# VISION-SJTU/VEON

Measured on AMD Instinct MI355X. Metric: 6cam_lift_samples_per_sec, higher is better.
Workload: dtype f32; 1 GPU; S2: 6-cam 256x704, D=59, C=80, 200x200x16 voxels, view_transform(accelerate=True) -> (B,C,Z,Y,X); points_kept=108978, intervals=72699, launch=eager, output_volume=allocator-placed (torch.empty per step), parallelism=replicas x1 (one sample per GPU, no collective)

## Files before the change

include/veon_hip.h:

```cpp
#ifndef VEON_HIP_H_
#define VEON_HIP_H_

#include <stddef.h>
#include <stdint.h>

#ifdef __cplusplus
extern "C" {
#endif

#define VEON_ABI_VERSION 2

#define VEON_OK 0
#define VEON_ERR_BAD_ARG 1
#define VEON_ERR_LAUNCH 2
#define VEON_ERR_WORKSPACE 3

#define VEON_LAYOUT_BZYXC 0
#define VEON_LAYOUT_BCZYX 1

#define VEON_FEAT_F32 0
#define VEON_FEAT_F16 1
#define VEON_FEAT_BF16 2


int veon_abi_version(void);
int veon_half_mode(void);
const char *veon_status_string(int status);

int veon_bev_pool_v2_fwd(int c, int n_intervals, const float *depth,
                         const float *feat, const int *ranks_depth,
                         const int *ranks_feat, const int *ranks_bev,
                         const int *interval_starts,
                         const int *interval_lengths, float *out, void *stream);

int veon_bev_pool_v2_bwd(int c, int n_intervals, const float *out_grad,
                         const float *depth, const float *feat,
                         const int *ranks_depth, const int *ranks_feat,
                         const int *ranks_bev, const int *interval_starts,
                         const int *interval_lengths, float *depth_grad,
                         float *feat_grad, void *stream);

int veon_bev_pool_tile_voxels(void);
int64_t veon_bev_pool_plan_ints(int batch, int64_t voxels_per_batch);
int veon_bev_pool_plan(int n_intervals, int n_points, int batch,
                       int64_t voxels_per_batch, const int *ranks_bev,
                       const int *interval_starts, const int *counts, int *plan,
                       void *stream);

int veon_bev_pool_v2_fwd_fused(int c, int n_intervals, int batch,
                               int64_t voxels_per_batch, const float *depth,
                               const float *feat, const int *ranks_depth,
                               const int *ranks_feat, const int *ranks_bev,
                               const int *interval_starts,
                               const int *interval_lengths, const int *plan,
                               float *out, int out_layout, void *stream);

int veon_bev_pool_row_table(int n_intervals, int n_points, int batch,
                            int64_t voxels_per_batch, int row_voxels,
                            const int *ranks_bev, const int *interval_starts,
                            const int *counts, int *row_first, int *row_point,
                            void *stream);
int veon_bev_pool_v2_fwd_maxpool(int c, int n_intervals, int batch, int Z, int Y,
                                 int X, int dz, int dy, int dx,
                                 const float *depth, const float *feat,
                                 const int *ranks_depth, const int *ranks_feat,
                                 const int *ranks_bev,
                                 const int *interval_starts,
                                 const int *interval_lengths,
                                 const int *row_first, float *out,
                                 void *stream);

int veon_bev_pool_v2_fwd_fused_ex(int c, int n_intervals, int batch,
                                  int64_t voxels_per_batch, const float *depth,
                                  const void *feat, int feat_dtype,
                                  const int *ranks_depth, const int *ranks_feat,
                                  const int *ranks_bev,
                                  const int *interval_starts,
                                  const int *interval_lengths, const int *plan,
                                  float *out, int out_layout, void *stream);
int veon_bev_pool_v2_fwd_maxpool_ex(int c, int n_intervals, int batch, int Z,
                                    int Y, int X, int dz, int dy, int dx,
                                    const float *depth, const void *feat,
                                    int feat_dtype, const int *ranks_depth,
                                    const int *ranks_feat, const int *ranks_bev,
                                    const int *interval_starts,
                                    const int *interval_lengths,
                                    const int *row_first, float *out,
                                    void *stream);

int veon_bev_pool_v2_fwd_fused_strided(int c, int n_intervals, int batch,
                                       int64_t voxels_per_batch, const float *depth,
                                       const void *feat, int feat_dtype,
                                       const int *ranks_depth, const int *ranks_feat,
                                       const int *ranks_bev,
                                       const int *interval_starts,
                                       const int *interval_lengths, const int *plan,
                                       float *out, int64_t plane_stride,
                                       void *stream);

int veon_feat_nchw_to_nhwc(const void *in, void *out, int elem_bytes, int images,
                           int C, int HW, void *stream);

int veon_bev_pool_v2_fwd_maxpool_padded(int c, int n_intervals, int batch, int Z,
                                        int Y, int X, int dz, int dy, int dx,
                                        const float *depth, const void *feat,
                                        int feat_dtype, const int *ranks_depth,
                                        const int *ranks_feat,
                                        const int *ranks_bev,
                                        const int *interval_starts,
                                        const int *interval_lengths,
                                        const int *row_first,
                                        void *out_padded_bf16, void *stream);

int veon_volume_maxpool2_f32(const float *in, float *out, int64_t planes, int Z, int Y,
                             int X, void *stream);


int64_t veon_bev_pool_voxel_table_ints(int batch, int64_t voxels_per_batch);
int veon_bev_pool_voxel_table(int n_intervals, int n_points, int batch,
                              int64_t voxels_per_batch, const int *ranks_bev,
                              const int *interval_starts, const int *counts,
                              int *vstart, void *stream);
int veon_bev_pool_v2_fwd_rows(int c, int batch, int64_t voxels_per_batch,
                              const float *depth, const void *feat, int feat_dtype,
                              const int *ranks_depth, const int *ranks_feat,
                              const int *vstart, float *out, int64_t plane_stride,
                              int64_t feat_elems, int variant, void *stream);
int veon_bev_pool_v2_fwd_rows_maxpool(int c, int batch, int Z, int Y, int X, int dz,
                                      int dy, int dx, const float *depth,
                                      const void *feat, int feat_dtype,
                                      const int *ranks_depth, const int *ranks_feat,
                                      const int *vstart, void *out, int out_padded_bf16,
                                      int64_t feat_elems, void *stream);

int veon_bev_pool_rows_maxpool_chunk(void);
int veon_bev_pool_v2_fwd_rows_maxpool_ordered(
    int c, int batch, int Z, int Y, int X, int dz, int dy, int dx, const float *depth,
    const void *feat, int feat_dtype, const int *ranks_depth, const int *ranks_feat,
    const int *vstart, void *out, int out_padded_bf16, int64_t feat_elems,
    const int *chunk_order, void *stream);

int veon_bev_pool_v2_fwd_rows_maxpool_winner(
    int c, int batch, int Z, int Y, int X, int dz, int dy, int dx, const float *depth,
    const void *feat, int feat_dtype, const int *ranks_depth, const int *ranks_feat,
    const int *vstart, void *out, int64_t feat_elems, const int *chunk_order,
    uint8_t *winner, void *stream);
int veon_bev_pool_point_table(int n_points, int64_t table_len, int64_t n_voxels,
                              const int *ranks_depth, const int *ranks_bev,
                              const int *counts, int *pvox, void *stream);
int veon_bev_pool_v2_bwd_rows_maxpool(int c, int n_images, int D, int HW, int batch, int Z,
                                      int Y, int X, const float *pooled_grad,
                                      const uint8_t *winner, const int *pvox,
                                      const float *depth, const float *feat,
                                      float *depth_grad, float *feat_grad, void *stream);


int veon_camera_matrices(int BN, const float *sensor2ego, const float *cam2imgs,
                         const float *post_rots, float *post_rots_inv,
                         float *combine, float *trans, void *stream);

int veon_lidar_coor(int B, int N, int D, int H, int W, const float *xs,
                    const float *ys, const float *ds,
                    const float *post_rots_inv, const float *post_trans,
                    const float *combine, const float *trans, const float *bda,
                    float *coor, void *stream);

int64_t veon_lss_prepare_workspace_bytes(int64_t num_points,
                                         int64_t num_voxels_total);
int veon_lss_prepare(int B, int N, int D, int H, int W, const float *coor,
                     const float *xs, const float *ys, const float *ds,
                     const float *post_rots_inv, const float *post_trans,
                     const float *combine, const float *trans, const float *bda,
                     const float *grid_lower, const float *grid_interval,
                     const float *grid_size, int64_t voxels_per_batch,
                     void *workspace, int64_t workspace_bytes, int *ranks_bev,
                     int *ranks_depth, int *ranks_feat, int *interval_starts,
                     int *interval_lengths, int *plan, int *counts,
                     void *stream);

int veon_lss_prepare_cameras(int B, int N, int D, int H, int W, const float *xs,
                             const float *ys, const float *ds,
                             const float *sensor2ego, const float *cam2imgs,
                             const float *post_rots, const float *post_trans,
                             const float *bda, const float *grid_lower,
                             const float *grid_interval, const float *grid_size,
                             int64_t voxels_per_batch, void *workspace,
                             int64_t workspace_bytes, int hist_is_zero,
                             int *ranks_bev, int *ranks_depth, int *ranks_feat,
                             int *interval_starts, int *interval_lengths, int *plan,
                             int *vstart, int *counts, void *stream);

int veon_lss_prepare_cameras_sparse(
    int B, int N, int D, int H, int W, const float *xs, const float *ys, const float *ds,
    const float *sensor2ego, const float *cam2imgs, const float *post_rots,
    const float *post_trans, const float *bda, const float *grid_lower,
    const float *grid_interval, const float *grid_size, int64_t voxels_per_batch,
    void *workspace, int64_t workspace_bytes, int hist_is_zero, int *ranks_bev,
    int *ranks_depth, int *ranks_feat, int *interval_starts, int *interval_lengths,
    int *plan, int *vstart, int *counts, const float *depth_weights, float depth_eps,
    void *stream);

int veon_lss_prepare_cameras_twohot(
    int B, int N, int D, int H, int W, const float *xs, const float *ys, const float *ds,
    const float *sensor2ego, const float *cam2imgs, const float *post_rots,
    const float *post_trans, const float *bda, const float *grid_lower,
    const float *grid_interval, const float *grid_size, int64_t voxels_per_batch,
    void *workspace, int64_t workspace_bytes, int hist_is_zero, int *ranks_bev,
    int *ranks_depth, int *ranks_feat, int *interval_starts, int *interval_lengths,
    int *plan, int *vstart, int *counts, const int *win, int window_slots, void *stream);

int veon_sensor2keyego(int B, int N, const float *sensor2ego, const float *ego2global,
                       float *out, void *stream);


int veon_downsample_depth(int BN, int H, int W, int ds, const float *depths,
                          float *out, void *stream);
int veon_two_hot_depth(int BN, int H, int W, int ds, int D, float lo, float step,
                       float gamma, const float *depths, float *out,
                       void *stream);

int veon_two_hot_window_slots(int D, float step, float gamma);
int veon_two_hot_window(int BN, int H, int W, int ds, int D, float lo, float step,
                        float gamma, float eps, int K, const float *depths, int *win,
                        float *wts, void *stream);


int veon_vit_cast_bf16(const float *in, void *out_bf16, int64_t n, void *stream);
int veon_vit_layernorm(const float *x, const float *gamma, const float *beta,
                       void *out_bf16, int T, int d, float eps, void *stream);
int veon_vit_gemm(const void *a_bf16, const void *w_bf16, const float *bias,
                  const float *gamma, float *resid, void *out_bf16, int M, int N,
                  int K, int epilogue, void *stream);
int veon_vit_attention(const void *qkv_bf16, const float *bias,
                       int64_t bias_batch_stride, int64_t bias_head_stride,
                       void *out_bf16, int B, int T, int H, int head_dim,
                       void *stream);
int veon_vit_attention_log2(const void *qkv_bf16, const float *bias,
                            int64_t bias_batch_stride, int64_t bias_head_stride,
                            void *out_bf16, int B, int T, int H, int head_dim,
                            void *stream);

int veon_vit_patchify(const float *img, void *out_bf16, int B, int C, int H, int W,
                      int patch, int skip, int kpad, void *stream);

int64_t veon_vit_gemm_splitk_plan(int M, int N, int K, int *tile_out);
int veon_vit_gemm_splitk(const void *a_bf16, const void *w_bf16, const float *bias,
                         const float *gamma, float *resid, int M, int N, int K,
                         void *slab, int64_t slab_bytes, int *sync_words,
                         int64_t sync_ints, void *stream);

typedef struct veon_vit_block_weights {
// ... 143 lines not shown
```

veon_amd/csrc/bev_pool_v2.hip:

```cpp
#include <hip/hip_runtime.h>
#include <stdint.h>

#include "../../include/veon_hip.h"
#include "half_mode.h"

extern "C" int veon_pool_debug_flags;

namespace {

constexpr int kBlock = 256;
constexpr int kWave = 64;

struct PoolArgs {
  const float* __restrict__ depth;
  const void* __restrict__ feat;
  const int* __restrict__ ranks_depth;
  const int* __restrict__ ranks_feat;
  const int* __restrict__ ranks_bev;
  const int* __restrict__ interval_starts;
  const int* __restrict__ interval_lengths;
};

template <int VEC>
struct Vec;
// ... 113 lines not shown
                    make_float4(bf_lo(u.z), bf_hi(u.z), bf_lo(u.w), bf_hi(u.w))};
    }
  }
}

template <int VEC, typename FT = FeatF32>
__device__ __forceinline__ typename Vec<VEC>::T interval_sum(
    const PoolArgs& a, int c, int start, int len, int ch) {
  using V = typename Vec<VEC>::T;
  V acc = vzero<VEC>();
  int i = 0;
  for (; i + 4 <= len; i += 4) {
    int rd[4], rf[4];
#pragma unroll
    for (int k = 0; k < 4; ++k) {
      rd[k] = a.ranks_depth[start + i + k];
      rf[k] = a.ranks_feat[start + i + k];
    }
    float d[4];
    V f[4];
#pragma unroll
    for (int k = 0; k < 4; ++k) {
      d[k] = a.depth[rd[k]];
      f[k] = load_feat<FT, VEC>(a.feat, (int64_t)rf[k] * c + ch);
    }
#pragma unroll
    for (int k = 0; k < 4; ++k) vfma<VEC>(acc, f[k], d[k]);
  }
  for (; i < len; ++i) {
    const int rd = a.ranks_depth[start + i];
    const int rf = a.ranks_feat[start + i];
    const float d = a.depth[rd];
    const V f = load_feat<FT, VEC>(a.feat, (int64_t)rf * c + ch);
    vfma<VEC>(acc, f, d);
  }
  return acc;
}

template <int VEC>
__global__ __launch_bounds__(kBlock) void k_pool_scatter(
    PoolArgs a, int c, int cq, int n_intervals, float* __restrict__ out) {
  const int64_t idx = (int64_t)blockIdx.x * kBlock + threadIdx.x;
  const int64_t interval = idx / cq;
  if (interval >= n_intervals) return;
  const int ch = (int)(idx - interval * cq) * VEC;
  const int start = a.interval_starts[interval];
  const int len = a.interval_lengths[interval];
  using V = typename Vec<VEC>::T;
  const V acc = interval_sum<VEC>(a, c, start, len, ch);
  *reinterpret_cast<V*>(out + (int64_t)a.ranks_bev[start] * c + ch) = acc;
}

constexpr int kTileV = 64;

__global__ __launch_bounds__(kBlock) void k_plan_bounds(
    const int* __restrict__ ranks_bev, const int* __restrict__ interval_starts,
    int n_intervals, int n_points, int64_t vpb, int64_t tiles_per_batch,
    int64_t n_tiles, int tile_voxels, int* __restrict__ tile_first,
    int* __restrict__ tile_point, const int* __restrict__ counts) {
  const int64_t i = (int64_t)blockIdx.x * kBlock + threadIdx.x;
  if (counts != nullptr) {
    n_points = counts[0];
    n_intervals = counts[1];
  }
  if (i > n_intervals) return;
  auto tile_of = [&](int rank) -> int64_t {
    const int64_t b = rank / vpb;
    return b * tiles_per_batch + (rank - b * vpb) / tile_voxels;
  };
  int64_t hi = n_tiles;
  int st = n_points;
  if (i < n_intervals) {
    st = interval_starts[i];
    hi = tile_of(ranks_bev[st]);
  }
  const int64_t lo =
      (i == 0) ? -1 : tile_of(ranks_bev[interval_starts[i - 1]]);
  for (int64_t tt = lo + 1; tt <= hi; ++tt) {
    tile_first[tt] = (int)i;
    tile_point[tt] = st;
  }
}

__global__ __launch_bounds__(kBlock) void k_plan_pack(
    const int* __restrict__ tile_first, const int* __restrict__ tile_point,
    int64_t n_tiles, int4* __restrict__ plan) {
  const int64_t t = (int64_t)blockIdx.x * kBlock + threadIdx.x;
  if (t >= n_tiles) return;
  plan[t] = make_int4(tile_first[t], tile_first[t + 1] - tile_first[t],
                      tile_point[t], tile_point[t + 1] - tile_point[t]);
}

struct TileInfo {
  int b;
  int64_t vox0;
  int nvox;
  int64_t rank0;
};

__device__ __forceinline__ TileInfo tile_info(int64_t t, int64_t tiles_per_batch,
                                              int64_t vpb) {
  TileInfo ti;
  ti.b = (int)(t / tiles_per_batch);
  ti.vox0 = (t - (int64_t)ti.b * tiles_per_batch) * kTileV;
  const int64_t rem = vpb - ti.vox0;
  ti.nvox = (int)(rem < kTileV ? rem : kTileV);
  ti.rank0 = (int64_t)ti.b * vpb + ti.vox0;
  return ti;
}

__device__ __forceinline__ unsigned long long wave_or(unsigned long long bit) {
  for (int off = 32; off > 0; off >>= 1) bit |= __shfl_xor(bit, off);
  return bit;
}

template <int VEC, typename FT>
__global__ __launch_bounds__(kBlock) void k_pool_fused_cl(
    PoolArgs a, const int4* __restrict__ plan, int c, int cq, int64_t vpb,
    int64_t tiles_per_batch, float* __restrict__ out) {
  const int64_t t = blockIdx.x;
  const TileInfo ti = tile_info(t, tiles_per_batch, vpb);
  const int4 pl = plan[t];
  const int i0 = pl.x, cnt = pl.y;
  using VT = typename Vec<VEC>::T;
  float* obase = out + ti.rank0 * c;
  const int items = ti.nvox * cq;
  if (cnt == 0) {
    for (int item = threadIdx.x; item < items; item += kBlock)
      reinterpret_cast<VT*>(obase)[item] = vzero<VEC>();
    return;
  }
  const int lane = threadIdx.x & (kWave - 1);
  unsigned long long bit = 0;
  if (lane < cnt)
    bit = 1ull << (int)((int64_t)a.ranks_bev[a.interval_starts[i0 + lane]] -
                        ti.rank0);
  const unsigned long long mask = wave_or(bit);
  for (int item = threadIdx.x; item < items; item += kBlock) {
    const int v = item / cq;
    const int ch = (item - v * cq) * VEC;
    VT acc = vzero<VEC>();
    if ((mask >> v) & 1ull) {
      const int ii = i0 + __popcll(mask & ((1ull << v) - 1ull));
      acc = interval_sum<VEC, FT>(a, c, a.interval_starts[ii],
                                  a.interval_lengths[ii], ch);
    }
    reinterpret_cast<VT*>(obase)[item] = acc;
  }
}

constexpr int kPmax = 1024;

template <int VEC, int CAP, typename FT>
__global__ __launch_bounds__(kBlock) void k_pool_fused_cf(
    PoolArgs a, const int4* __restrict__ plan, int c, int cs, int64_t vpb,
    int64_t tiles_per_batch, float* __restrict__ out, int64_t ostride, int chunked) {
  extern __shared__ float lds[];
  constexpr int LDC = CAP + 1;
  constexpr int UNROLL = 8;
  constexpr int SB = 5;
  constexpr int NW = kBlock / kWave;
  float* tile = lds;
  int* istart = reinterpret_cast<int*>(lds + (size_t)cs * LDC);
  int* ivox = istart + kTileV + 2;
  int* s_rf = ivox + kTileV;
  int* s_rd = s_rf + kPmax;

  const int tid = threadIdx.x;
  const int lane = tid & (kWave - 1);
  const int w = tid >> 6;
  int64_t t = blockIdx.x;
  if (chunked >= 0) {
    const int64_t sg = t >> (3 + chunked);
    if (((sg + 1) << (3 + chunked)) <= (int64_t)gridDim.x)
      t = (((sg << 3) + (t & 7)) << chunked) + ((t >> 3) & ((1 << chunked) - 1));
  }
  const int c0 = blockIdx.y * cs;
  const int nch = (c - c0) < cs ? (c - c0) : cs;
  const TileInfo ti = tile_info(t, tiles_per_batch, vpb);
  float* obase = out + ((int64_t)ti.b * c + c0) * ostride + ti.vox0;

  const int4 pl = plan[t];
  const int i0 = pl.x, cnt = pl.y, p0 = pl.z, npts = pl.w;

  if (cnt == 0) {
    if (lane < ti.nvox)
      for (int cc = w; cc < nch; cc += NW)
        __builtin_nontemporal_store(0.f, obase + (int64_t)cc * ostride + lane);
    return;
  }
  if (tid < cnt) {
    const int st = a.interval_starts[i0 + tid];
    istart[tid] = st - p0;
    ivox[tid] = (int)((int64_t)a.ranks_bev[st] - ti.rank0);
  }
  if (tid == 0) istart[cnt] = npts;
  {
    const int n = npts < kPmax ? npts : kPmax;
    for (int p = tid; p < n; p += kBlock) {
      s_rf[p] = a.ranks_feat[p0 + p];
      s_rd[p] = a.ranks_depth[p0 + p];
    }
  }
  __syncthreads();

  const unsigned long long mask =
      wave_or(lane < cnt ? (1ull << ivox[lane]) : 0ull);
  using VT = typename Vec<VEC>::T;
  const int nq = nch / VEC;
  const int npass = cnt > CAP ? 2 : 1;
  const int jsplit = __popcll(mask & 0xffffffffull);
  int base = 0;
  for (int pass = 0; pass < npass; ++pass) {
    const int ja = (npass == 2 && pass == 1) ? jsplit : 0;
    const int jb = (npass == 2 && pass == 0) ? jsplit : cnt;
    int j0 = ja;
    while (j0 < jb) {
      int j1 = j0;
      while (j1 < jb && istart[j1 + 1] - base <= kPmax) ++j1;
      if (j1 == j0) {
        const int st = istart[j0];
        const int len = istart[j0 + 1] - st;
        if (len > kPmax) {
          for (int q = tid; q < nq; q += kBlock) {
            const VT acc =
                interval_sum<VEC, FT>(a, c, p0 + st, len, c0 + q * VEC);
            const float* ap = reinterpret_cast<const float*>(&acc);
#pragma unroll
            for (int k = 0; k < VEC; ++k)
              tile[(q * VEC + k) * LDC + (j0 - ja)] = ap[k];
          }
          ++j0;
          continue;
        }
        __syncthreads();
        base = st;
        const int n = (npts - base) < kPmax ? (npts - base) : kPmax;
        for (int p = tid; p < n; p += kBlock) {
          s_rf[p] = a.ranks_feat[p0 + base + p];
          s_rd[p] = a.ranks_depth[p0 + base + p];
        }
        __syncthreads();
        continue;
      }
      const int items = (j1 - j0) * nq;
      for (int item = tid; item < items; item += kBlock) {
        const int j = j0 + item / nq;
        const int q = item - (j - j0) * nq;
        const int st = istart[j] - base;
        const int len = istart[j + 1] - istart[j];
        const int64_t fcol = c0 + q * VEC;
        VT acc = vzero<VEC>();
        int i = 0;
        for (; i + UNROLL <= len; i += UNROLL) {
          VT f[UNROLL];
          float d[UNROLL];
#pragma unroll
          for (int u = 0; u < UNROLL; ++u) {
            f[u] = load_feat<FT, VEC>(a.feat,
                                      fcol + (int64_t)s_rf[st + i + u] * c);
            d[u] = a.depth[s_rd[st + i + u]];
          }
#pragma unroll
          for (int u = 0; u < UNROLL; ++u) vfma<VEC>(acc, f[u], d[u]);
        }
        for (; i < len; ++i) {
          const VT f =
              load_feat<FT, VEC>(a.feat, fcol + (int64_t)s_rf[st + i] * c);
          vfma<VEC>(acc, f, a.depth[s_rd[st + i]]);
        }
        const float* ap = reinterpret_cast<const float*>(&acc);
#pragma unroll
        for (int k = 0; k < VEC; ++k)
          tile[(q * VEC + k) * LDC + (j - ja)] = ap[k];
      }
      j0 = j1;
    }
    __syncthreads();
    if (npass == 1) {
      const bool occupied = (mask >> lane) & 1ull;
      const int col = __popcll(mask & ((1ull << lane) - 1ull));
      if (lane < ti.nvox) {
        float* op = obase + lane;
        int cc = w;
        for (; cc + (SB - 1) * NW < nch; cc += SB * NW) {
          float vals[SB];
#pragma unroll
          for (int u = 0; u < SB; ++u)
            vals[u] = occupied ? tile[(cc + NW * u) * LDC + col] : 0.f;
#pragma unroll
          for (int u = 0; u < SB; ++u)
            __builtin_nontemporal_store(vals[u],
                                        op + (int64_t)(cc + NW * u) * ostride);
        }
        for (; cc < nch; cc += NW)
          __builtin_nontemporal_store(occupied ? tile[cc * LDC + col] : 0.f,
                                      op + (int64_t)cc * ostride);
      }
    } else {
      const int v = pass * 32 + (lane & 31);
      const bool occupied = (mask >> v) & 1ull;
      const int col = __popcll(mask & ((1ull << v) - 1ull)) - ja;
      if (v < ti.nvox)
        for (int cc = 2 * w + (lane >> 5); cc < nch; cc += 2 * NW)
          __builtin_nontemporal_store(occupied ? tile[cc * LDC + col] : 0.f,
                                      obase + (int64_t)cc * ostride + v);
      if (pass == 0) __syncthreads();
    }
  }
}

__device__ __forceinline__ int float_key(float f) {
  const int b = __float_as_int(f);
  return b ^ ((b >> 31) & 0x7fffffff);
}
__device__ __forceinline__ float key_float(int k) {
  return __int_as_float(k ^ ((k >> 31) & 0x7fffffff));
}

template <int VEC, typename FT, bool PADDED = false>
__global__ __launch_bounds__(kBlock) void k_pool_maxpool_cf(
    PoolArgs a, const int* __restrict__ row_first, int c, int cs, int Z, int Y,
    int X, int dz, int dy, int dx, float* __restrict__ out) {
  extern __shared__ int ldsi[];
  const int Zo = Z / dz, Yo = Y / dy, Xo = X / dx;
  int* tile = ldsi;
  int* occ = ldsi + cs * Xo;
  const int tid = threadIdx.x;
  const int64_t orow = blockIdx.x;
  const int yo = (int)(orow % Yo);
  const int zo = (int)((orow / Yo) % Zo);
  const int b = (int)(orow / ((int64_t)Yo * Zo));
  const int c0 = blockIdx.y * cs;
  const int nch = (c - c0) < cs ? (c - c0) : cs;
  const int nq = nch / VEC;
  const int kmin = float_key(-__builtin_inff());
  for (int i = tid; i < cs * Xo; i += kBlock) tile[i] = kmin;
  for (int i = tid; i < Xo; i += kBlock) occ[i] = 0;
  __syncthreads();
  using VT = typename Vec<VEC>::T;
  for (int rz = 0; rz < dz; ++rz)
    for (int ry = 0; ry < dy; ++ry) {
      const int64_t row = ((int64_t)b * Z + (zo * dz + rz)) * Y + (yo * dy + ry);
      const int64_t rank0 = row * X;
      const int i0 = row_first[row];
      const int cnt = row_first[row + 1] - i0;
      const int items = cnt * nq;
      for (int item = tid; item < items; item += kBlock) {
        const int j = item / nq;
        const int q = item - j * nq;
        const int start = a.interval_starts[i0 + j];
        const int len = a.interval_lengths[i0 + j];
        const int xo = (int)((int64_t)a.ranks_bev[start] - rank0) / dx;
        const VT acc = interval_sum<VEC, FT>(a, c, start, len, c0 + q * VEC);
        const float* ap = reinterpret_cast<const float*>(&acc);
#pragma unroll
        for (int k = 0; k < VEC; ++k)
          atomicMax(&tile[(q * VEC + k) * Xo + xo], float_key(ap[k]));
        if (q == 0) atomicAdd(&occ[xo], 1);
      }
    }
  __syncthreads();
  const int full = dz * dy * dx;
  if constexpr (PADDED) {
    unsigned short* ob =
        reinterpret_cast<unsigned short*>(out) +
        ((((int64_t)b * (Zo + 2) + zo + 1) * (Yo + 2) + yo + 1) * (Xo + 2) + 1) *
            (int64_t)c + c0;
    for (int i = tid; i < nch * Xo; i += kBlock) {
      const int xo = i / nch;
      const int cc = i - xo * nch;
      const int n = occ[xo];
      float v = 0.f;
      if (n > 0) {
        v = key_float(tile[cc * Xo + xo]);
        if (n < full && !(v > 0.f)) v = 0.f;
      }
      ob[(int64_t)xo * c + cc] = __builtin_bit_cast(unsigned short, (veon_half_native)v);
    }
    return;
  }
  float* obase =
      out + ((((int64_t)b * c + c0) * Zo + zo) * Yo + yo) * (int64_t)Xo;
  const int64_t cstride = (int64_t)Zo * Yo * Xo;
  for (int i = tid; i < nch * Xo; i += kBlock) {
    const int cc = i / Xo;
    const int xo = i - cc * Xo;
    const int n = occ[xo];
    float v = 0.f;
    if (n > 0) {
      v = key_float(tile[cc * Xo + xo]);
      if (n < full && !(v > 0.f)) v = 0.f;
    }
    obase[(int64_t)cc * cstride + xo] = v;
  }
}

constexpr int kBwdBlock = 128;

template <int VEC>
__global__ __launch_bounds__(kBwdBlock) void k_pool_bwd(
    PoolArgs a, int c, int n_intervals, const float* __restrict__ out_grad,
    float* __restrict__ depth_grad, float* __restrict__ feat_grad) {
  const int interval = blockIdx.x;
  const int start = a.interval_starts[interval];
  const int len = a.interval_lengths[interval];
  using VT = typename Vec<VEC>::T;
  for (int i = threadIdx.x; i < len; i += kBwdBlock) {
    const float* og = out_grad + (int64_t)a.ranks_bev[start + i] * c;
    const float* ft =
        static_cast<const float*>(a.feat) + (int64_t)a.ranks_feat[start + i] * c;
    float s = 0.f;
    for (int cc = 0; cc < c; cc += VEC) {
      const VT o = *reinterpret_cast<const VT*>(og + cc);
      const VT f = *reinterpret_cast<const VT*>(ft + cc);
      if constexpr (VEC == 4) {
        s = fmaf(o.x, f.x, s);
        s = fmaf(o.y, f.y, s);
        s = fmaf(o.z, f.z, s);
        s = fmaf(o.w, f.w, s);
      } else {
        s = fmaf(o, f, s);
      }
    }
    depth_grad[a.ranks_depth[start + i]] = s;
  }
  float* fg = feat_grad + (int64_t)a.ranks_feat[start] * c;
  for (int cc = threadIdx.x; cc < c; cc += kBwdBlock) {
    float s = 0.f;
    for (int i = 0; i < len; ++i) {
      const float og = out_grad[(int64_t)a.ranks_bev[start + i] * c + cc];
      s = fmaf(og, a.depth[a.ranks_depth[start + i]], s);
    }
    fg[cc] = s;
  }
}

inline int launch_status() {
  return hipGetLastError() == hipSuccess ? VEON_OK : VEON_ERR_LAUNCH;
}

inline bool aligned16(const void* p) {
  return (reinterpret_cast<uintptr_t>(p) & 15u) == 0;
}

}

namespace {
template <typename T>
__global__ __launch_bounds__(256) void k_feat_nchw_to_nhwc(const T* __restrict__ in,
                                                           T* __restrict__ out, int C,
                                                           int HW) {
  __shared__ T t[64][65];
  const int p0 = blockIdx.x * 64, c0 = blockIdx.y * 64;
  const T* ib = in + (int64_t)blockIdx.z * C * HW;
  T* ob = out + (int64_t)blockIdx.z * HW * C;
  const int tx = threadIdx.x & 63, ty = threadIdx.x >> 6;
  T v[16];
#pragma unroll
  for (int k = 0; k < 16; ++k) {
    const int c = c0 + ty + 4 * k, p = p0 + tx;
// ... 133 lines not shown
      !plan)
    return VEON_ERR_BAD_ARG;
  if (n_intervals > 0 && (!ranks_bev || !interval_starts))
    return VEON_ERR_BAD_ARG;
  if ((reinterpret_cast<uintptr_t>(plan) & 15u) != 0) return VEON_ERR_BAD_ARG;
  const int64_t tiles_per_batch = (voxels_per_batch + kTileV - 1) / kTileV;
  const int64_t n_tiles = tiles_per_batch * batch;
  if (n_tiles > 0x3fffffffLL) return VEON_ERR_BAD_ARG;
  int* tile_first = plan + 4 * n_tiles;
  int* tile_point = tile_first + (n_tiles + 1);
  hipStream_t s = static_cast<hipStream_t>(stream);
  const unsigned b1 = (unsigned)(((int64_t)n_intervals + 1 + kBlock - 1) / kBlock);
  hipLaunchKernelGGL(k_plan_bounds, dim3(b1), dim3(kBlock), 0, s, ranks_bev,
                     interval_starts, n_intervals, n_points, voxels_per_batch,
                     tiles_per_batch, n_tiles, kTileV, tile_first, tile_point, counts);
  const unsigned b2 = (unsigned)((n_tiles + kBlock - 1) / kBlock);
  hipLaunchKernelGGL(k_plan_pack, dim3(b2), dim3(kBlock), 0, s, tile_first,
                     tile_point, n_tiles, reinterpret_cast<int4*>(plan));
  return launch_status();
}

int veon_bev_pool_row_table(int n_intervals, int n_points, int batch,
                            int64_t voxels_per_batch, int row_voxels,
                            const int* ranks_bev, const int* interval_starts,
                            const int* counts, int* row_first, int* row_point,
                            void* stream) {
  if (n_intervals < 0 || n_points < 0 || batch <= 0 || voxels_per_batch <= 0 ||
      row_voxels <= 0 || voxels_per_batch % row_voxels != 0 || !row_first ||
      !row_point)
    return VEON_ERR_BAD_ARG;
  if (n_intervals > 0 && (!ranks_bev || !interval_starts))
    return VEON_ERR_BAD_ARG;
  const int64_t rows_per_batch = voxels_per_batch / row_voxels;
  const int64_t n_rows = rows_per_batch * batch;
  if (n_rows > 0x3fffffffLL) return VEON_ERR_BAD_ARG;
  const unsigned b1 = (unsigned)(((int64_t)n_intervals + 1 + kBlock - 1) / kBlock);
  hipLaunchKernelGGL(k_plan_bounds, dim3(b1), dim3(kBlock), 0,
                     static_cast<hipStream_t>(stream), ranks_bev,
                     interval_starts, n_intervals, n_points, voxels_per_batch,
                     rows_per_batch, n_rows, row_voxels, row_first, row_point, counts);
  return launch_status();
}

static int maxpool_impl(bool padded, int c, int n_intervals, int batch, int Z,
                                    int Y, int X, int dz, int dy, int dx,
                                    const float* depth, const void* feat,
                                    int feat_dtype, const int* ranks_depth,
                                    const int* ranks_feat, const int* ranks_bev,
                                    const int* interval_starts,
                                    const int* interval_lengths,
                                    const int* row_first, float* out,
                                    void* stream) {
  if (c <= 0 || n_intervals < 0 || batch <= 0 || Z <= 0 || Y <= 0 || X <= 0 ||
      dz <= 0 || dy <= 0 || dx <= 0 || Z % dz || Y % dy || X % dx || !out ||
      !row_first)
    return VEON_ERR_BAD_ARG;
  if (feat_dtype != VEON_FEAT_F32 && feat_dtype != VEON_FEAT_F16 &&
      feat_dtype != VEON_FEAT_BF16)
    return VEON_ERR_BAD_ARG;
  if (n_intervals > 0 &&
      (!depth || !feat || !ranks_depth || !ranks_feat || !ranks_bev ||
       !interval_starts || !interval_lengths))
    return VEON_ERR_BAD_ARG;
  if ((int64_t)batch * Z * Y * X > 0x7fffffffLL) return VEON_ERR_BAD_ARG;
  PoolArgs a{depth, feat, ranks_depth, ranks_feat, ranks_bev, interval_starts,
             interval_lengths};
  const int Xo = X / dx;
  int cs = c;
  while ((int64_t)cs * Xo * 4 > 16384 && cs > 8) cs = (cs / 2 + 7) / 8 * 8;
  const int slabs = (c + cs - 1) / cs;
  const size_t lds = ((size_t)cs * Xo + Xo) * sizeof(int);
  const int64_t orows = (int64_t)batch * (Z / dz) * (Y / dy);
  if (orows > 0x7fffffffLL) return VEON_ERR_BAD_ARG;
  const dim3 grid((unsigned)orows, (unsigned)slabs);
  hipStream_t s = static_cast<hipStream_t>(stream);
#define VEON_LAUNCH_MP(VEC, FT)                                               \
  do {                                                                        \
    if (padded)                                                               \
      hipLaunchKernelGGL((k_pool_maxpool_cf<VEC, FT, true>), grid,            \
                         dim3(kBlock), lds, s, a, row_first, c, cs, Z, Y, X,  \
                         dz, dy, dx, out);                                    \
    else                                                                      \
      hipLaunchKernelGGL((k_pool_maxpool_cf<VEC, FT, false>), grid,           \
                         dim3(kBlock), lds, s, a, row_first, c, cs, Z, Y, X,  \
                         dz, dy, dx, out);                                    \
  } while (0)
  if (feat_dtype == VEON_FEAT_F32) {
    if ((c % 4 == 0) && (cs % 4 == 0) && aligned16(feat))
      VEON_LAUNCH_MP(4, FeatF32);
    else
      VEON_LAUNCH_MP(1, FeatF32);
  } else {
    const bool v4 = (c % 4 == 0) && (cs % 4 == 0) && aligned16(feat);
    const bool v8 = v4 && (c % 8 == 0) && (cs % 8 == 0) && c >= 128;
    if (feat_dtype == VEON_FEAT_F16) {
      if (v8) VEON_LAUNCH_MP(8, FeatF16);
      else if (v4) VEON_LAUNCH_MP(4, FeatF16);
      else VEON_LAUNCH_MP(1, FeatF16);
    } else {
      if (v8) VEON_LAUNCH_MP(8, FeatBF16);
      else if (v4) VEON_LAUNCH_MP(4, FeatBF16);
      else VEON_LAUNCH_MP(1, FeatBF16);
    }
  }
#undef VEON_LAUNCH_MP
  return launch_status();
}

int veon_bev_pool_v2_fwd_maxpool_ex(int c, int n_intervals, int batch, int Z,
                                    int Y, int X, int dz, int dy, int dx,
                                    const float* depth, const void* feat,
                                    int feat_dtype, const int* ranks_depth,
                                    const int* ranks_feat, const int* ranks_bev,
                                    const int* interval_starts,
                                    const int* interval_lengths,
                                    const int* row_first, float* out,
                                    void* stream) {
  return maxpool_impl(false, c, n_intervals, batch, Z, Y, X, dz, dy, dx, depth,
                      feat, feat_dtype, ranks_depth, ranks_feat, ranks_bev,
                      interval_starts, interval_lengths, row_first, out, stream);
}

int veon_bev_pool_v2_fwd_maxpool_padded(int c, int n_intervals, int batch, int Z,
                                        int Y, int X, int dz, int dy, int dx,
                                        const float* depth, const void* feat,
                                        int feat_dtype, const int* ranks_depth,
                                        const int* ranks_feat,
                                        const int* ranks_bev,
                                        const int* interval_starts,
                                        const int* interval_lengths,
                                        const int* row_first,
                                        void* out_padded_bf16, void* stream) {
  return maxpool_impl(true, c, n_intervals, batch, Z, Y, X, dz, dy, dx, depth,
                      feat, feat_dtype, ranks_depth, ranks_feat, ranks_bev,
                      interval_starts, interval_lengths, row_first,
                      static_cast<float*>(out_padded_bf16), stream);
}

int veon_bev_pool_v2_fwd_maxpool(int c, int n_intervals, int batch, int Z, int Y,
                                 int X, int dz, int dy, int dx,
                                 const float* depth, const float* feat,
                                 const int* ranks_depth, const int* ranks_feat,
                                 const int* ranks_bev,
                                 const int* interval_starts,
                                 const int* interval_lengths,
                                 const int* row_first, float* out,
                                 void* stream) {
  return veon_bev_pool_v2_fwd_maxpool_ex(
      c, n_intervals, batch, Z, Y, X, dz, dy, dx, depth, feat, VEON_FEAT_F32,
      ranks_depth, ranks_feat, ranks_bev, interval_starts, interval_lengths,
      row_first, out, stream);
}

static int fused_impl(int c, int n_intervals, int batch, int64_t voxels_per_batch,
                      const float* depth, const void* feat, int feat_dtype,
                      const int* ranks_depth, const int* ranks_feat,
                      const int* ranks_bev, const int* interval_starts,
                      const int* interval_lengths, const int* plan, float* out,
                      int out_layout, int64_t plane_stride, void* stream) {
  if (c <= 0 || n_intervals < 0 || batch <= 0 || voxels_per_batch <= 0 ||
      !out || !plan)
    return VEON_ERR_BAD_ARG;
  if (plane_stride == 0) plane_stride = voxels_per_batch;
  if (plane_stride < voxels_per_batch ||
      (plane_stride != voxels_per_batch && out_layout != VEON_LAYOUT_BCZYX))
    return VEON_ERR_BAD_ARG;
  if (out_layout != VEON_LAYOUT_BZYXC && out_layout != VEON_LAYOUT_BCZYX)
    return VEON_ERR_BAD_ARG;
  if (feat_dtype != VEON_FEAT_F32 && feat_dtype != VEON_FEAT_F16 &&
      feat_dtype != VEON_FEAT_BF16)
    return VEON_ERR_BAD_ARG;
  if (n_intervals > 0 &&
      (!depth || !feat || !ranks_depth || !ranks_feat || !ranks_bev ||
       !interval_starts || !interval_lengths))
    return VEON_ERR_BAD_ARG;
  if ((int64_t)batch * voxels_per_batch > 0x7fffffffLL)
    return VEON_ERR_BAD_ARG;
  if ((reinterpret_cast<uintptr_t>(plan) & 15u) != 0) return VEON_ERR_BAD_ARG;
  PoolArgs a{depth, feat, ranks_depth, ranks_feat, ranks_bev, interval_starts,
             interval_lengths};
  hipStream_t s = static_cast<hipStream_t>(stream);
  const int64_t tiles_per_batch = (voxels_per_batch + kTileV - 1) / kTileV;
  const int64_t n_tiles = tiles_per_batch * batch;
  if (n_tiles > 0x3fffffffLL) return VEON_ERR_BAD_ARG;
  const int4* plan4 = reinterpret_cast<const int4*>(plan);
  if (out_layout == VEON_LAYOUT_BZYXC) {
    const bool v4 = (c % 4 == 0) && aligned16(feat) && aligned16(out);
#define VEON_LAUNCH_CL(VEC, FT)                                                \
  hipLaunchKernelGGL((k_pool_fused_cl<VEC, FT>), dim3((unsigned)n_tiles),      \
                     dim3(kBlock), 0, s, a, plan4, c, c / VEC,                 \
                     voxels_per_batch, tiles_per_batch, out)
    if (feat_dtype == VEON_FEAT_F32) {
      if (v4) VEON_LAUNCH_CL(4, FeatF32); else VEON_LAUNCH_CL(1, FeatF32);
    } else if (feat_dtype == VEON_FEAT_F16) {
      if (v4) VEON_LAUNCH_CL(4, FeatF16); else VEON_LAUNCH_CL(1, FeatF16);
    } else {
      if (v4) VEON_LAUNCH_CL(4, FeatBF16); else VEON_LAUNCH_CL(1, FeatBF16);
    }
#undef VEON_LAUNCH_CL
    return launch_status();
  }
  const int cs = c <= 128 ? c : 64;
  const int slabs = (c + cs - 1) / cs;
  const bool dense = (int64_t)n_intervals > 12 * n_tiles;
  const int cap = dense ? 64 : 32;
  const size_t lds = (size_t)cs * (cap + 1) * sizeof(float) +
                     (size_t)(2 * kTileV + 2 + 2 * kPmax) * sizeof(int);
  const dim3 grid((unsigned)n_tiles, (unsigned)slabs);
  const int ov = (veon_pool_debug_flags >> 8) & 15;
  const int chunked = (slabs != 1 || (veon_pool_debug_flags & 16)) ? -1 : (ov ? ov - 1 : -1);
#define VEON_LAUNCH_CF(VEC, CAP, FT)                                          \
  hipLaunchKernelGGL((k_pool_fused_cf<VEC, CAP, FT>), grid, dim3(kBlock), lds, \
                     s, a, plan4, c, cs, voxels_per_batch, tiles_per_batch, out,   \
                     plane_stride, chunked)
#define VEON_LAUNCH_CF2(VEC, FT) \
  do { if (dense) VEON_LAUNCH_CF(VEC, 64, FT); else VEON_LAUNCH_CF(VEC, 32, FT); } while (0)
  if (feat_dtype == VEON_FEAT_F32) {
    if ((c % 4 == 0) && aligned16(feat)) VEON_LAUNCH_CF2(4, FeatF32);
    else VEON_LAUNCH_CF2(1, FeatF32);
  } else {
    const bool v4 = (c % 4 == 0) && (cs % 4 == 0) && aligned16(feat);
    if (feat_dtype == VEON_FEAT_F16) {
      if (v4) VEON_LAUNCH_CF2(4, FeatF16); else VEON_LAUNCH_CF2(1, FeatF16);
    } else {
      if (v4) VEON_LAUNCH_CF2(4, FeatBF16); else VEON_LAUNCH_CF2(1, FeatBF16);
    }
  }
#undef VEON_LAUNCH_CF2
#undef VEON_LAUNCH_CF
  return launch_status();
}

int veon_bev_pool_v2_fwd_fused_ex(int c, int n_intervals, int batch,
                                  int64_t voxels_per_batch, const float* depth,
                                  const void* feat, int feat_dtype,
                                  const int* ranks_depth, const int* ranks_feat,
                                  const int* ranks_bev,
                                  const int* interval_starts,
                                  const int* interval_lengths, const int* plan,
                                  float* out, int out_layout, void* stream) {
  return fused_impl(c, n_intervals, batch, voxels_per_batch, depth, feat, feat_dtype,
                    ranks_depth, ranks_feat, ranks_bev, interval_starts,
                    interval_lengths, plan, out, out_layout, 0, stream);
}

int veon_bev_pool_v2_fwd_fused_strided(int c, int n_intervals, int batch,
                                       int64_t voxels_per_batch, const float* depth,
                                       const void* feat, int feat_dtype,
                                       const int* ranks_depth, const int* ranks_feat,
                                       const int* ranks_bev,
                                       const int* interval_starts,
                                       const int* interval_lengths, const int* plan,
                                       float* out, int64_t plane_stride,
                                       void* stream) {
  return fused_impl(c, n_intervals, batch, voxels_per_batch, depth, feat, feat_dtype,
                    ranks_depth, ranks_feat, ranks_bev, interval_starts,
                    interval_lengths, plan, out, VEON_LAYOUT_BCZYX, plane_stride,
                    stream);
}

int veon_bev_pool_v2_fwd_fused(int c, int n_intervals, int batch,
                               int64_t voxels_per_batch, const float* depth,
                               const float* feat, const int* ranks_depth,
                               const int* ranks_feat, const int* ranks_bev,
                               const int* interval_starts,
                               const int* interval_lengths, const int* plan,
                               float* out, int out_layout, void* stream) {
  return veon_bev_pool_v2_fwd_fused_ex(
      c, n_intervals, batch, voxels_per_batch, depth, feat, VEON_FEAT_F32,
      ranks_depth, ranks_feat, ranks_bev, interval_starts, interval_lengths,
      plan, out, out_layout, stream);
}

int veon_feat_nchw_to_nhwc(const void* in, void* out, int elem_bytes, int images,
                           int C, int HW, void* stream) {
  if (!in || !out || in == out || images <= 0 || C <= 0 || HW <= 0 ||
      (elem_bytes != 4 && elem_bytes != 2) || images > 65535)
    return VEON_ERR_BAD_ARG;
  const dim3 grid((unsigned)((HW + 63) / 64), (unsigned)((C + 63) / 64), (unsigned)images);
  hipStream_t s = static_cast<hipStream_t>(stream);
  if (elem_bytes == 4)
    hipLaunchKernelGGL(k_feat_nchw_to_nhwc<float>, grid, dim3(256), 0, s,
                       static_cast<const float*>(in), static_cast<float*>(out), C, HW);
  else
    hipLaunchKernelGGL(k_feat_nchw_to_nhwc<unsigned short>, grid, dim3(256), 0, s,
                       static_cast<const unsigned short*>(in),
                       static_cast<unsigned short*>(out), C, HW);
  return launch_status();
}

int veon_volume_maxpool2_f32(const float* in, float* out, int64_t planes, int Z, int Y,
                             int X, void* stream) {
  if (!in || !out || planes <= 0 || Z <= 0 || Y <= 0 || X <= 0 || (Z & 1) || (Y & 1) || (X & 1))
    return VEON_ERR_BAD_ARG;
  const int64_t total = planes * (Z / 2) * (Y / 2) * (X / 2);
  const int64_t blocks = (total + 255) / 256;
  if (blocks > 0x7fffffffLL) return VEON_ERR_BAD_ARG;
  hipLaunchKernelGGL(k_volume_maxpool2, dim3((unsigned)blocks), dim3(256), 0,
                     static_cast<hipStream_t>(stream), in, out, planes, Z, Y, X);
  return launch_status();
}

}
```

Baseline: 22670 samples/s.

## Add persistent large-LDS fused BEV pool kernel batching many tiles per workgroup

Adds a persistent channel-first fused pooling kernel that launches one 1024-thread workgroup per CU. Each workgroup batches up to 64 tiles at a time, staging interval metadata, feature ranks and depths in a large LDS arena, and flattens interval-by-channel work across all threads before writing the zero-filled output planes. The goal is to cut per-tile launch and scheduling overhead and the load imbalance of the one-block-per-tile slab kernel, and to raise memory-level parallelism through unrolled staged gathers. The cost is a single fat workgroup per CU with heavy LDS use and serialized phases, which may lower occupancy and latency hiding.

After: 19260 samples/s. -15.0%, worse.

```diff
diff --git a/include/veon_hip.h b/include/veon_hip.h
--- a/include/veon_hip.h
+++ b/include/veon_hip.h
@@ -97,6 +97,11 @@
                                        const int *interval_lengths, const int *plan,
                                        float *out, int64_t plane_stride,
                                        void *stream);
+
+#define VEON_POOL_FUSED_SLAB 0
+#define VEON_POOL_FUSED_PERSISTENT 1
+int veon_bev_pool_fused_variant(int c, int batch, int64_t voxels_per_batch,
+                                int out_layout);
 
 int veon_feat_nchw_to_nhwc(const void *in, void *out, int elem_bytes, int images,
                            int C, int HW, void *stream);
diff --git a/veon_amd/csrc/bev_pool_v2.hip b/veon_amd/csrc/bev_pool_v2.hip
--- a/veon_amd/csrc/bev_pool_v2.hip
+++ b/veon_amd/csrc/bev_pool_v2.hip
@@ -289,7 +289,7 @@
 constexpr int kPmax = 1024;
 
 template <int VEC, int CAP, typename FT>
-__global__ __launch_bounds__(kBlock) void k_pool_fused_cf(
+__global__ __launch_bounds__(kBlock) void k_pool_slab_cf(
     PoolArgs a, const int4* __restrict__ plan, int c, int cs, int64_t vpb,
     int64_t tiles_per_batch, float* __restrict__ out, int64_t ostride, int chunked) {
   extern __shared__ float lds[];
@@ -444,6 +444,211 @@
                                       obase + (int64_t)cc * ostride + v);
       if (pass == 0) __syncthreads();
     }
+  }
+}
+
+constexpr int kPThreads = 1024;
+constexpr int kPWgPerCu = 1;
+constexpr int kPTiles = 64;
+constexpr int kPIntervals = 512;
+constexpr int kPPoints = 2048;
+constexpr int kPU = 16;
+constexpr bool kPStoreSc1 = false;
+constexpr int kPFixedWords = 4 + 10 * kPTiles + 4 * kPIntervals + 2 * kPPoints;
+
+__device__ __forceinline__ int wave_scan_incl(int v, int lane) {
+  for (int off = 1; off < kWave; off <<= 1) {
+    const int o = __shfl_up(v, off);
+    if (lane >= off) v += o;
+  }
+  return v;
+}
+
+__device__ __forceinline__ int last_le(const int* tab, int n, int x) {
+  int lo = 0, hi = n;
+  while (hi - lo > 1) {
+    const int mid = (lo + hi) >> 1;
+    if (tab[mid] <= x) lo = mid; else hi = mid;
+  }
+  return lo;
+}
+
+__device__ __forceinline__ void pool_store(float* p, float v) {
+  if constexpr (kPStoreSc1)
+    __hip_atomic_store(p, v, __ATOMIC_RELAXED, __HIP_MEMORY_SCOPE_AGENT);
+  else
+    *p = v;
+}
+
+template <int VEC, typename FT, int U>
+__device__ __forceinline__ void staged_trip(typename Vec<VEC>::T& acc, const void* feat,
+                                            int64_t fcol, int c, const int* s_rf,
+                                            const float* s_d, int at, int n) {
+  using VT = typename Vec<VEC>::T;
+  VT f[U];
+  if (n == U) {
+#pragma unroll
+    for (int u = 0; u < U; ++u)
+      f[u] = load_feat<FT, VEC>(feat, fcol + (int64_t)s_rf[at + u] * c);
+#pragma unroll
+    for (int u = 0; u < U; ++u) vfma<VEC>(acc, f[u], s_d[at + u]);
+  } else {
+#pragma unroll
+    for (int u = 0; u < U; ++u)
+      if (u < n) f[u] = load_feat<FT, VEC>(feat, fcol + (int64_t)s_rf[at + u] * c);
+#pragma unroll
+    for (int u = 0; u < U; ++u)
+      if (u < n) vfma<VEC>(acc, f[u], s_d[at + u]);
+  }
+}
+
+template <int VEC, typename FT>
+__global__ __launch_bounds__(kPThreads) void k_pool_fused_cf(
+    PoolArgs a, const int4* __restrict__ plan, int c, int64_t vpb,
+    int64_t tiles_per_batch, int64_t n_tiles, float* __restrict__ out,
+    int64_t ostride, int arena_floats) {
+  extern __shared__ float lds[];
+  constexpr int NW = kPThreads / kWave;
+  constexpr int SB = 5;
+  int* s_hdr = reinterpret_cast<int*>(lds);
+  int4* s_plan = reinterpret_cast<int4*>(s_hdr + 4);
+  unsigned long long* s_mask =
+      reinterpret_cast<unsigned long long*>(s_plan + kPTiles);
+  int* s_toff = reinterpret_cast<int*>(s_mask + kPTiles);
+  int* s_tj = s_toff + kPTiles;
+  int* s_tp = s_tj + kPTiles;
+  int* s_tb = s_tp + kPTiles;
+  int* s_ist = s_tb + kPTiles;
+  int* s_ilen = s_ist + kPIntervals;
+  int* s_idst = s_ilen + kPIntervals;
+  int* s_ivox = s_idst + kPIntervals;
+  int* s_rf = s_ivox + kPIntervals;
+  float* s_d = reinterpret_cast<float*>(s_rf + kPPoints);
+  float* arena = s_d + kPPoints;
+
+  const int tid = threadIdx.x;
+  const int lane = tid & (kWave - 1);
+  const int wv = tid >> 6;
+  const int64_t n_wg = gridDim.x;
+  const int64_t first = blockIdx.x;
+  using VT = typename Vec<VEC>::T;
+  const int nq = c / VEC;
+
+  for (int64_t kbase = 0; first + kbase * n_wg < n_tiles;) {
+    if (wv == 0) {
+      const int64_t t = first + (kbase + lane) * n_wg;
+      const bool valid = t < n_tiles;
+      const int4 pl = valid ? plan[t] : make_int4(0, 0, 0, 0);
+      const int ldc = pl.y | 1;
+      const int need = pl.y > 0 ? c * ldc : 0;
+      const int pts = pl.w <= kPPoints ? pl.w : 0;
+      const int e_need = wave_scan_incl(need, lane);
+      const int e_cnt = wave_scan_incl(pl.y, lane);
+      const int e_pts = wave_scan_incl(pts, lane);
+      const bool fits = valid && e_need <= arena_floats && e_cnt <= kPIntervals &&
+                        e_pts <= kPPoints;
+      const unsigned long long miss = ~__ballot(fits);
+      const int nt = miss ? __ffsll((long long)miss) - 1 : kWave;
+      if (lane < nt) {
+        s_plan[lane] = pl;
+        s_toff[lane] = e_need - need;
+        s_tj[lane] = e_cnt - pl.y;
+        s_tp[lane] = e_pts - pts;
+        s_tb[lane] = (int)(t / tiles_per_batch);
+      }
+      if (lane == (nt > 0 ? nt - 1 : 0)) {
+        s_hdr[0] = nt;
+        s_hdr[1] = nt > 0 ? e_cnt : 0;
+        s_hdr[2] = nt > 0 ? e_pts : 0;
+      }
+    }
+    __syncthreads();
+    const int nt = s_hdr[0], ni = s_hdr[1], np = s_hdr[2];
+    if (nt == 0) return;
+
+    for (int jj = tid; jj < ni; jj += kPThreads) {
+      const int k = last_le(s_tj, nt, jj);
+      const int4 pl = s_plan[k];
+      const int j = jj - s_tj[k];
+      const int st = a.interval_starts[pl.x + j];
+      const int en = (j + 1 < pl.y) ? a.interval_starts[pl.x + j + 1] : pl.z + pl.w;
+      const int64_t t = first + (kbase + k) * n_wg;
+      const int64_t rank0 =
+          (int64_t)s_tb[k] * vpb + (t - (int64_t)s_tb[k] * tiles_per_batch) * kTileV;
+      s_ivox[jj] = (int)((int64_t)a.ranks_bev[st] - rank0);
+      s_ist[jj] = pl.w <= kPPoints ? s_tp[k] + (st - pl.z) : -1 - st;
+      s_ilen[jj] = en - st;
+      s_idst[jj] = (s_toff[k] + j) | ((pl.y | 1) << 20);
+    }
+    for (int pp = tid; pp < np; pp += kPThreads) {
+      const int k = last_le(s_tp, nt, pp);
+      const int p = s_plan[k].z + (pp - s_tp[k]);
+      s_rf[pp] = a.ranks_feat[p];
+      s_d[pp] = a.depth[a.ranks_depth[p]];
+    }
+    __syncthreads();
+
+    for (int k = wv; k < nt; k += NW) {
+      const int cnt = s_plan[k].y;
+      const unsigned long long m =
+          wave_or(lane < cnt ? (1ull << s_ivox[s_tj[k] + lane]) : 0ull);
+      if (lane == 0) s_mask[k] = m;
+    }
+    const int items = ni * nq;
+    for (int item = tid; item < items; item += kPThreads) {
+      const int jj = item / nq;
+      const int q = item - jj * nq;
+      const int at = s_ist[jj];
+      const int len = s_ilen[jj];
+      VT acc = vzero<VEC>();
+      if (at < 0) {
+        acc = interval_sum<VEC, FT>(a, c, -1 - at, len, q * VEC);
+      } else {
+        const int64_t fcol = q * VEC;
+        int i = 0;
+        for (; i + kPU <= len; i += kPU)
+          staged_trip<VEC, FT, kPU>(acc, a.feat, fcol, c, s_rf, s_d, at + i, kPU);
+        const int rem = len - i;
+        if (rem > kPU / 2)
+          staged_trip<VEC, FT, kPU>(acc, a.feat, fcol, c, s_rf, s_d, at + i, rem);
+        else if (rem > 0)
+          staged_trip<VEC, FT, kPU / 2>(acc, a.feat, fcol, c, s_rf, s_d, at + i, rem);
+      }
+      const int dst = s_idst[jj];
+      const int ldc = dst >> 20;
+      float* tp = arena + (dst & 0xfffff) + q * VEC * ldc;
+      const float* ap = reinterpret_cast<const float*>(&acc);
+#pragma unroll
+      for (int k = 0; k < VEC; ++k) tp[k * ldc] = ap[k];
+    }
+    __syncthreads();
+
+    for (int k = 0; k < nt; ++k) {
+      const int cnt = s_plan[k].y;
+      const int b = s_tb[k];
+      const int64_t vox0 = (first + (kbase + k) * n_wg - (int64_t)b * tiles_per_batch) * kTileV;
+      const int64_t rem = vpb - vox0;
+      if (lane >= (rem < kTileV ? rem : kTileV)) continue;
+      float* op = out + (int64_t)b * c * ostride + vox0 + lane;
+      const unsigned long long mask = cnt > 0 ? s_mask[k] : 0ull;
+      const bool occupied = (mask >> lane) & 1ull;
+      const int ldc = cnt | 1;
+      const float* tp = arena + s_toff[k] + __popcll(mask & ((1ull << lane) - 1ull));
+      int cc = wv;
+      for (; cc + (SB - 1) * NW < c; cc += SB * NW) {
+        float vals[SB];
+#pragma unroll
+        for (int u = 0; u < SB; ++u)
+          vals[u] = occupied ? tp[(cc + NW * u) * ldc] : 0.f;
+#pragma unroll
+        for (int u = 0; u < SB; ++u)
+          pool_store(op + (int64_t)(cc + NW * u) * ostride, vals[u]);
+      }
+      for (; cc < c; cc += NW)
+        pool_store(op + (int64_t)cc * ostride, occupied ? tp[cc * ldc] : 0.f);
+    }
+    kbase += nt;
+    __syncthreads();
   }
 }
 
@@ -883,6 +1088,51 @@
       row_first, out, stream);
 }
 
+static bool persistent_limits(int* n_cu, int* lds_bytes) {
+  constexpr int kMaxDev = 64;
+  static int cu[kMaxDev], lds[kMaxDev];
+  int dev = 0;
+  if (hipGetDevice(&dev) != hipSuccess || dev < 0 || dev >= kMaxDev) {
+    (void)hipGetLastError();
+    return false;
+  }
+  if (cu[dev] == 0) {
+    int n = 0, l = 0, per_cu = 0;
+    if (hipDeviceGetAttribute(&n, hipDeviceAttributeMultiprocessorCount, dev) != hipSuccess ||
+        hipDeviceGetAttribute(&l, hipDeviceAttributeMaxSharedMemoryPerBlock, dev) != hipSuccess ||
+        n <= 0 || l <= 0) {
+      (void)hipGetLastError();
+      return false;
+    }
+    if (hipDeviceGetAttribute(&per_cu, hipDeviceAttributeMaxSharedMemoryPerMultiprocessor,
+                              dev) == hipSuccess && per_cu > l)
+      l = per_cu;
+    (void)hipGetLastError();
+    lds[dev] = l < 160 * 1024 ? l : 160 * 1024;
+    cu[dev] = n;
+  }
+  *n_cu = cu[dev];
+  *lds_bytes = lds[dev];
+  return true;
+}
+
+constexpr int kPMinTilesPerCu = 4;
+
+static int fused_variant(int c, int64_t n_tiles, int out_layout) {
+  if (out_layout != VEON_LAYOUT_BCZYX || c > 128) return VEON_POOL_FUSED_SLAB;
+  int n_cu = 0, lds_bytes = 0;
+  if (!persistent_limits(&n_cu, &lds_bytes)) return VEON_POOL_FUSED_SLAB;
+  return n_tiles >= (int64_t)kPMinTilesPerCu * n_cu ? VEON_POOL_FUSED_PERSISTENT
+                                                    : VEON_POOL_FUSED_SLAB;
+}
+
+int veon_bev_pool_fused_variant(int c, int batch, int64_t voxels_per_batch,
+                                int out_layout) {
+  if (c <= 0 || batch <= 0 || voxels_per_batch <= 0) return VEON_POOL_FUSED_SLAB;
+  const int64_t n_tiles = ((voxels_per_batch + kTileV - 1) / kTileV) * batch;
+  return fused_variant(c, n_tiles, out_layout);
+}
+
 static int fused_impl(int c, int n_intervals, int batch, int64_t voxels_per_batch,
                       const float* depth, const void* feat, int feat_dtype,
                       const int* ranks_depth, const int* ranks_feat,
@@ -931,6 +1181,35 @@
 #undef VEON_LAUNCH_CL
     return launch_status();
   }
+  if (fused_variant(c, n_tiles, out_layout) == VEON_POOL_FUSED_PERSISTENT) {
+    int n_cu = 0, lds_bytes = 0;
+    if (!persistent_limits(&n_cu, &lds_bytes)) return VEON_ERR_LAUNCH;
+    const int lds = lds_bytes / kPWgPerCu;
+    const int arena_floats = lds / (int)sizeof(float) - kPFixedWords;
+    if (arena_floats < c * (kTileV + 1)) return VEON_ERR_LAUNCH;
+    const int64_t want = (int64_t)n_cu * kPWgPerCu;
+    const unsigned n_wg = (unsigned)(want < n_tiles ? want : n_tiles);
+#define VEON_LAUNCH_PCF(VEC, FT)                                                  \
+  do {                                                                            \
+    static const hipError_t attr = hipFuncSetAttribute(                           \
+        reinterpret_cast<const void*>(&k_pool_fused_cf<VEC, FT>),                 \
+        hipFuncAttributeMaxDynamicSharedMemorySize, lds);                         \
+    if (attr != hipSuccess) return VEON_ERR_LAUNCH;                               \
+    hipLaunchKernelGGL((k_pool_fused_cf<VEC, FT>), dim3(n_wg), dim3(kPThreads),   \
+                       (size_t)lds, s, a, plan4, c, voxels_per_batch,             \
+                       tiles_per_batch, n_tiles, out, plane_stride, arena_floats); \
+  } while (0)
+    const bool v4 = (c % 4 == 0) && aligned16(feat);
+    if (feat_dtype == VEON_FEAT_F32) {
+      if (v4) VEON_LAUNCH_PCF(4, FeatF32); else VEON_LAUNCH_PCF(1, FeatF32);
+    } else if (feat_dtype == VEON_FEAT_F16) {
+      if (v4) VEON_LAUNCH_PCF(4, FeatF16); else VEON_LAUNCH_PCF(1, FeatF16);
+    } else {
+      if (v4) VEON_LAUNCH_PCF(4, FeatBF16); else VEON_LAUNCH_PCF(1, FeatBF16);
+    }
+#undef VEON_LAUNCH_PCF
+    return launch_status();
+  }
   const int cs = c <= 128 ? c : 64;
   const int slabs = (c + cs - 1) / cs;
   const bool dense = (int64_t)n_intervals > 12 * n_tiles;
@@ -941,7 +1220,7 @@
   const int ov = (veon_pool_debug_flags >> 8) & 15;
   const int chunked = (slabs != 1 || (veon_pool_debug_flags & 16)) ? -1 : (ov ? ov - 1 : -1);
 #define VEON_LAUNCH_CF(VEC, CAP, FT)                                          \
-  hipLaunchKernelGGL((k_pool_fused_cf<VEC, CAP, FT>), grid, dim3(kBlock), lds, \
+  hipLaunchKernelGGL((k_pool_slab_cf<VEC, CAP, FT>), grid, dim3(kBlock), lds,  \
                      s, a, plan4, c, cs, voxels_per_batch, tiles_per_batch, out,   \
                      plane_stride, chunked)
 #define VEON_LAUNCH_CF2(VEC, FT) \
```
